# PersiaML/PERSIA

Hardware: AMD Instinct MI355X
Metric: samples/sec (whole node), DLRM-style hybrid training (higher is better)
Workload: dtype bf16; 1 GPU; preset=criteo, model=dlrm 26sparse/13dense dim128, global_batch=8192, rows=100000000, capacity_per_rank=100000000, staleness=8, parallelism=dp1+emb-a2a

## Files before the change

### persia_amd/csrc/dense.hip

```cpp
#include <torch/extension.h>
#include <ATen/hip/HIPContext.h>
#include <hip/hip_runtime.h>
#include <hip/hip_bf16.h>

using bf16 = __hip_bfloat16;
using f32x4 = __attribute__((ext_vector_type(4))) float;
using bf16x8 = __attribute__((ext_vector_type(8))) short;

namespace {

constexpr int BM = 128, BN = 128, BK = 32;
constexpr int PAD = 8;
constexpr int LDK = BK + PAD;

__device__ __forceinline__ float bf2f(short x) {
  union { float f; unsigned u; } v;
  v.u = ((unsigned)(unsigned short)x) << 16;
  return v.f;
}

__device__ __forceinline__ short f2bf(float f) {
  union { float f; unsigned u; } v;
  v.f = f;
  unsigned lsb = (v.u >> 16) & 1;
  v.u += 0x7fff + lsb;
  return (short)(v.u >> 16);
}

template <int ACT, bool STORE_F32, bool TRANS_B, int TBN, int TBK>
__global__ __launch_bounds__(256) void gemm_nt_kernel(
    const bf16* __restrict__ A, const bf16* __restrict__ B,
    const float* __restrict__ bias, void* __restrict__ C, int M, int N,
    int K) {
  constexpr int LK = TBK + PAD;
  __shared__ short lds_a[2][BM * LK];
  __shared__ short lds_b[2][TBN * LK];
  constexpr int WN = TBN / 2;
  constexpr int NFRAG = WN / 16;
  constexpr int PA = BM * TBK / (256 * 8);
  constexpr int PB = TBN * TBK / (256 * 8);
  constexpr int ACPR = TBK / 8;

  const int n_tiles_n = (N + TBN - 1) / TBN;
  const int m0 = (blockIdx.x / n_tiles_n) * BM;
  const int n0 = (blockIdx.x % n_tiles_n) * TBN;

  const int tid = threadIdx.x;
  const int lane = tid % 64;
  const int wave = tid / 64;
  const int wr = wave / 2, wc = wave % 2;
  const int fi = lane & 15;
  const int fk8 = (lane >> 4) * 8;

  f32x4 acc[4][NFRAG] = {};

  auto stage_load = [&](int k0, bf16x8 (&ra)[PA], bf16x8 (&rb)[PB]) {
#pragma unroll
    for (int i = 0; i < PA; ++i) {
      const int p = tid + i * 256;
      const int r = p / ACPR, c8 = (p % ACPR) * 8;
      ra[i] = bf16x8{};
      if (m0 + r < M)
        ra[i] = *(const bf16x8*)(A + (int64_t)(m0 + r) * K + k0 + c8);
    }
#pragma unroll
    for (int i = 0; i < PB; ++i) {
      const int p = tid + i * 256;
      rb[i] = bf16x8{};
      if (!TRANS_B) {
        const int r = p / ACPR, c8 = (p % ACPR) * 8;
        if (n0 + r < N)
          rb[i] = *(const bf16x8*)(B + (int64_t)(n0 + r) * K + k0 + c8);
      } else {
        const int r = p / (TBN / 8), c8 = (p % (TBN / 8)) * 8;
        if (n0 + c8 < N)
          rb[i] = *(const bf16x8*)(B + (int64_t)(k0 + r) * N + n0 + c8);
      }
    }
  };
  auto bswz = [](int n, int k) {
    return n * LK +
           ((((k >> 3) ^ ((n >> 3) & (TBK / 8 - 1))) << 3) | (k & 7));
  };
  auto stage_write = [&](int buf, bf16x8 (&ra)[PA], bf16x8 (&rb)[PB]) {
#pragma unroll
    for (int i = 0; i < PA; ++i) {
      const int p = tid + i * 256;
      const int r = p / ACPR, c8 = (p % ACPR) * 8;
      *(bf16x8*)&lds_a[buf][r * LK + c8] = ra[i];
    }
#pragma unroll
    for (int i = 0; i < PB; ++i) {
      const int p = tid + i * 256;
      if (!TRANS_B) {
        const int r = p / ACPR, c8 = (p % ACPR) * 8;
        *(bf16x8*)&lds_b[buf][bswz(r, c8)] = rb[i];
      } else {
        const int r = p / (TBN / 8), c8 = (p % (TBN / 8)) * 8;
#pragma unroll
        for (int j = 0; j < 8; ++j)
          lds_b[buf][bswz(c8 + j, r)] = rb[i][j];
      }
    }
  };

  int buf = 0;
  {
    bf16x8 ra[PA], rb[PB];
    stage_load(0, ra, rb);
    stage_write(0, ra, rb);
  }
  __syncthreads();

  for (int k0 = 0; k0 < K; k0 += TBK) {
    bf16x8 ra[PA], rb[PB];
    const bool prefetch = k0 + TBK < K;
    if (prefetch) stage_load(k0 + TBK, ra, rb);
#pragma unroll
    for (int kk = 0; kk < TBK; kk += 32) {
#pragma unroll
      for (int am = 0; am < 4; ++am) {
        const bf16x8 a_frag = *(const bf16x8*)
            &lds_a[buf][(wr * 64 + am * 16 + fi) * LK + kk + fk8];
#pragma unroll
        for (int bn = 0; bn < NFRAG; ++bn) {
          const bf16x8 b_frag = *(const bf16x8*)
              &lds_b[buf][bswz(wc * WN + bn * 16 + fi, kk + fk8)];
          acc[am][bn] = __builtin_amdgcn_mfma_f32_16x16x32_bf16(
              a_frag, b_frag, acc[am][bn], 0, 0, 0);
        }
      }
    }
    if (prefetch) stage_write(buf ^ 1, ra, rb);
    buf ^= 1;
    __syncthreads();
  }

#pragma unroll
  for (int am = 0; am < 4; ++am) {
#pragma unroll
    for (int bn = 0; bn < NFRAG; ++bn) {
      const int col = n0 + wc * WN + bn * 16 + fi;
      if (col >= N) continue;
      const float bval = bias ? bias[col] : 0.0f;
#pragma unroll
      for (int r = 0; r < 4; ++r) {
        const int row = m0 + wr * 64 + am * 16 + (lane >> 4) * 4 + r;
        if (row >= M) continue;
        float v = acc[am][bn][r] + bval;
        if (ACT == 1) v = fmaxf(v, 0.0f);
        if (STORE_F32)
          ((float*)C)[(int64_t)row * N + col] = v;
        else
          ((short*)C)[(int64_t)row * N + col] = f2bf(v);
      }
    }
  }
}

using bf16x4t = __attribute__((ext_vector_type(4))) __bf16;

__global__ __launch_bounds__(256) void wgrad_tr_kernel(
    const short* __restrict__ dC, const short* __restrict__ A,
    float* __restrict__ dW, int M, int N, int K, int splitm, int ldw,
    int kmax, int accum) {
  constexpr int MT = 64;
  __shared__ short lds_c[2][8 * MT * 16];
  __shared__ short lds_a[2][8 * MT * 16];
  const int n_tiles_k = K / 128;
  const int tile_id = blockIdx.x / splitm;
  const int m_part = blockIdx.x % splitm;
  const int n0 = (tile_id / n_tiles_k) * 128;
  const int k0 = (tile_id % n_tiles_k) * 128;
  const int tid = threadIdx.x;
  const int wave = tid / 64, lane = tid % 64;
  const int wr = wave / 2, wc = wave % 2;
  const int fi = lane & 15;

  const int m_chunk = ((M + splitm - 1) / splitm + MT - 1) / MT * MT;
  const int m_begin = m_part * m_chunk;
  const int m_end = min(M, m_begin + m_chunk);

  const int s_m = lane >> 1;
  const int s_n8 = (lane & 1) * 8;
  auto stage = [&](int bufi, int m0g) {
#pragma unroll
    for (int c = 0; c < 4; ++c) {
      const int p = wave * 2 + (c >> 1);
      const int mrow = (c & 1) * 32 + s_m;
      const int64_t m_g = (int64_t)(m0g + mrow);
      __builtin_amdgcn_global_load_lds(
          (const uint32_t*)(dC + m_g * N + n0 + p * 16 + s_n8),
          (uint32_t*)&lds_c[bufi][(p * MT + (c & 1) * 32) * 16], 16, 0, 0);
      __builtin_amdgcn_global_load_lds(
          (const uint32_t*)(A + m_g * K + k0 + p * 16 + s_n8),
          (uint32_t*)&lds_a[bufi][(p * MT + (c & 1) * 32) * 16], 16, 0, 0);
    }
  };
  const int t_l4 = (lane & 15) * 4;
  const int t_g8 = (lane >> 4) * 8;
  auto tfrag = [&](const short* img, int p, int ms) {
    const short* b0 = &img[(p * MT + ms + t_g8) * 16 + t_l4];
    bf16x4t lo = __builtin_amdgcn_ds_read_tr16_b64_v4bf16(
        (__attribute__((address_space(3))) bf16x4t*)(void*)const_cast<short*>(b0));
    bf16x4t hi = __builtin_amdgcn_ds_read_tr16_b64_v4bf16(
        (__attribute__((address_space(3))) bf16x4t*)(void*)const_cast<short*>(b0 + 4 * 16));
    bf16x8 r;
#pragma unroll
    for (int j = 0; j < 4; ++j) {
      r[j] = ((const short*)&lo)[j];
      r[4 + j] = ((const short*)&hi)[j];
    }
    return r;
  };

  f32x4 acc[4][4] = {};
  stage(0, m_begin);
  asm volatile("s_waitcnt vmcnt(0)" ::: "memory");
  __builtin_amdgcn_s_barrier();
  int buf = 0;
  for (int m0g = m_begin; m0g < m_end; m0g += MT) {
    if (m0g + MT < m_end) stage(buf ^ 1, m0g + MT);
#pragma unroll
    for (int ms = 0; ms < MT; ms += 32) {
      bf16x8 bfr[4];
#pragma unroll
      for (int bk = 0; bk < 4; ++bk)
        bfr[bk] = tfrag(lds_a[buf], wc * 4 + bk, ms);
#pragma unroll
      for (int an = 0; an < 4; ++an) {
        const bf16x8 afr = tfrag(lds_c[buf], wr * 4 + an, ms);
#pragma unroll
        for (int bk = 0; bk < 4; ++bk)
          acc[an][bk] = __builtin_amdgcn_mfma_f32_16x16x32_bf16(
              afr, bfr[bk], acc[an][bk], 0, 0, 0);
      }
    }
    asm volatile("s_waitcnt vmcnt(0) lgkmcnt(0)" ::: "memory");
    __builtin_amdgcn_s_barrier();
    buf ^= 1;
  }

#pragma unroll
  for (int an = 0; an < 4; ++an) {
#pragma unroll
    for (int bk = 0; bk < 4; ++bk) {
      const int n = n0 + wr * 64 + an * 16 + (lane >> 4) * 4;
      const int k = k0 + wc * 64 + bk * 16 + fi;
      if (k >= kmax) continue;
#pragma unroll
      for (int r = 0; r < 4; ++r) {
        if (accum || splitm > 1)
          atomicAdd(&dW[(int64_t)(n + r) * ldw + k], acc[an][bk][r]);
        else
          dW[(int64_t)(n + r) * ldw + k] = acc[an][bk][r];
      }
    }
  }
}

template <int ACT, bool STORE_F32, int TBN>
__global__ __launch_bounds__(256) void gemm_nt_glds_kernel(
    const bf16* __restrict__ A, const bf16* __restrict__ B,
    const float* __restrict__ bias, void* __restrict__ C, int M, int N,
    int K) {
  constexpr int TBK = 64;
  constexpr int WN = TBN / 2;
  constexpr int NFRAG = WN / 16;
  constexpr int BCH = TBN / 32;
  __shared__ short lds_a[2][128 * TBK];
  __shared__ short lds_b[2][TBN * TBK];
  const int n_tiles_n = N / TBN;
  const int m0 = (blockIdx.x / n_tiles_n) * 128;
  const int n0 = (blockIdx.x % n_tiles_n) * TBN;
  const int tid = threadIdx.x;
  const int lane = tid % 64;
  const int wave = tid / 64;
  const int wr = wave / 2, wc = wave % 2;
  const int fi = lane & 15;
  const int g16 = lane >> 4;

  const int s_rl = lane >> 3;
  const int s_gr = (lane & 7) ^ s_rl;
  auto stage = [&](int bufi, int k0) {
#pragma unroll
    for (int i = 0; i < 4; ++i) {
      const int row = wave * 32 + i * 8 + s_rl;
      const int a_row = min(m0 + row, M - 1);
      __builtin_amdgcn_global_load_lds(
          (const uint32_t*)(A + (int64_t)a_row * K + k0 + s_gr * 8),
          (uint32_t*)&lds_a[bufi][(wave * 32 + i * 8) * TBK], 16, 0, 0);
    }
#pragma unroll
    for (int i = 0; i < BCH; ++i) {
      const int brow = wave * (TBN / 4) + i * 8 + s_rl;
      __builtin_amdgcn_global_load_lds(
          (const uint32_t*)(B + (int64_t)(n0 + brow) * K + k0 + s_gr * 8),
          (uint32_t*)&lds_b[bufi][(wave * (TBN / 4) + i * 8) * TBK], 16, 0, 0);
    }
  };
  auto frag = [&](const short* base, int row, int gr) {
    return *(const bf16x8*)&base[row * TBK + ((gr ^ (row & 7)) << 3)];
  };

  f32x4 acc[4][NFRAG] = {};
  stage(0, 0);
  asm volatile("s_waitcnt vmcnt(0)" ::: "memory");
  __builtin_amdgcn_s_barrier();
  int buf = 0;
  for (int k0 = 0; k0 < K; k0 += TBK) {
    if (k0 + TBK < K) stage(buf ^ 1, k0 + TBK);
#pragma unroll
    for (int kk = 0; kk < 2; ++kk) {
      bf16x8 bfr[NFRAG];
#pragma unroll
      for (int bn = 0; bn < NFRAG; ++bn)
        bfr[bn] = frag(lds_b[buf], wc * WN + bn * 16 + fi, kk * 4 + g16);
#pragma unroll
      for (int am = 0; am < 4; ++am) {
        const bf16x8 afr = frag(lds_a[buf], wr * 64 + am * 16 + fi,
                                kk * 4 + g16);
#pragma unroll
        for (int bn = 0; bn < NFRAG; ++bn)
          acc[am][bn] = __builtin_amdgcn_mfma_f32_16x16x32_bf16(
              afr, bfr[bn], acc[am][bn], 0, 0, 0);
      }
    }
    asm volatile("s_waitcnt vmcnt(0) lgkmcnt(0)" ::: "memory");
    __builtin_amdgcn_s_barrier();
    buf ^= 1;
  }

#pragma unroll
  for (int am = 0; am < 4; ++am) {
#pragma unroll
    for (int bn = 0; bn < NFRAG; ++bn) {
      const int col = n0 + wc * WN + bn * 16 + fi;
      const float bval = bias ? bias[col] : 0.0f;
#pragma unroll
      for (int r = 0; r < 4; ++r) {
        const int row = m0 + wr * 64 + am * 16 + (lane >> 4) * 4 + r;
        if (row >= M) continue;
        float v = acc[am][bn][r] + bval;
        if (ACT == 1) v = fmaxf(v, 0.0f);
        if (STORE_F32)
          ((float*)C)[(int64_t)row * N + col] = v;
        else
          ((short*)C)[(int64_t)row * N + col] = f2bf(v);
      }
    }
  }
}

template <int ACT, bool STORE_F32>
__global__ __launch_bounds__(256) void gemm_nt_glds3_kernel(
    const bf16* __restrict__ A, const bf16* __restrict__ B,
    const float* __restrict__ bias, void* __restrict__ C, int M, int N,
    int K) {
  constexpr int TBK = 64;
  __shared__ short lds_a[3][128 * TBK];
  __shared__ short lds_b[3][128 * TBK];
  const int n_tiles_n = N / 128;
  const int m0 = (blockIdx.x / n_tiles_n) * 128;
  const int n0 = (blockIdx.x % n_tiles_n) * 128;
  const int tid = threadIdx.x;
  const int lane = tid % 64;
  const int wave = tid / 64;
  const int wr = wave / 2, wc = wave % 2;
  const int fi = lane & 15;
  const int g16 = lane >> 4;
  const int s_rl = lane >> 3;
  const int s_gr = (lane & 7) ^ s_rl;
  auto stage = [&](int bufi, int k0) {
#pragma unroll
    for (int i = 0; i < 4; ++i) {
      const int row = wave * 32 + i * 8 + s_rl;
      const int a_row = min(m0 + row, M - 1);
      __builtin_amdgcn_global_load_lds(
          (const uint32_t*)(A + (int64_t)a_row * K + k0 + s_gr * 8),
          (uint32_t*)&lds_a[bufi][(wave * 32 + i * 8) * TBK], 16, 0, 0);
      __builtin_amdgcn_global_load_lds(
          (const uint32_t*)(B + (int64_t)(n0 + row) * K + k0 + s_gr * 8),
          (uint32_t*)&lds_b[bufi][(wave * 32 + i * 8) * TBK], 16, 0, 0);
    }
  };
  auto frag = [&](const short* base, int row, int gr) {
    return *(const bf16x8*)&base[row * TBK + ((gr ^ (row & 7)) << 3)];
  };

  f32x4 acc[4][4] = {};
  const int nt = K / TBK;
  stage(0, 0);
  if (nt > 1) {
    stage(1, TBK);
    asm volatile("s_waitcnt vmcnt(8)" ::: "memory");
  } else {
    asm volatile("s_waitcnt vmcnt(0)" ::: "memory");
  }
  __builtin_amdgcn_s_barrier();
  for (int t = 0; t < nt; ++t) {
    if (t + 2 < nt) stage((t + 2) % 3, (t + 2) * TBK);
    const short* la = lds_a[t % 3];
    const short* lb = lds_b[t % 3];
#pragma unroll
    for (int kk = 0; kk < 2; ++kk) {
      bf16x8 bfr[4];
#pragma unroll
      for (int bn = 0; bn < 4; ++bn)
        bfr[bn] = frag(lb, wc * 64 + bn * 16 + fi, kk * 4 + g16);
#pragma unroll
      for (int am = 0; am < 4; ++am) {
        const bf16x8 afr = frag(la, wr * 64 + am * 16 + fi, kk * 4 + g16);
#pragma unroll
        for (int bn = 0; bn < 4; ++bn)
          acc[am][bn] = __builtin_amdgcn_mfma_f32_16x16x32_bf16(
              afr, bfr[bn], acc[am][bn], 0, 0, 0);
      }
    }
    if (t + 2 < nt)
      asm volatile("s_waitcnt vmcnt(8) lgkmcnt(0)" ::: "memory");
    else
      asm volatile("s_waitcnt vmcnt(0) lgkmcnt(0)" ::: "memory");
    __builtin_amdgcn_s_barrier();
  }

#pragma unroll
  for (int am = 0; am < 4; ++am) {
#pragma unroll
    for (int bn = 0; bn < 4; ++bn) {
      const int col = n0 + wc * 64 + bn * 16 + fi;
      const float bval = bias ? bias[col] : 0.0f;
#pragma unroll
      for (int r = 0; r < 4; ++r) {
        const int row = m0 + wr * 64 + am * 16 + (lane >> 4) * 4 + r;
        if (row >= M) continue;
        float v = acc[am][bn][r] + bval;
        if (ACT == 1) v = fmaxf(v, 0.0f);
        if (STORE_F32)
          ((float*)C)[(int64_t)row * N + col] = v;
        else
          ((short*)C)[(int64_t)row * N + col] = f2bf(v);
      }
    }
  }
}

constexpr int WTM = 64;
constexpr int WLD = WTM + PAD;

__global__ __launch_bounds__(256) void wgrad_kernel(
    const short* __restrict__ dC, const short* __restrict__ A,
    float* __restrict__ dW, int M, int N, int K, int splitm, int ldw,
    int kmax, int accum) {
  __shared__ short lds_dct[2][64 * WLD];
  __shared__ short lds_at[2][64 * WLD];

  const int n_tiles_k = (K + 63) / 64;
  const int tile_id = blockIdx.x / splitm;
  const int m_part = blockIdx.x % splitm;
  const int n0 = (tile_id / n_tiles_k) * 64;
  const int k0 = (tile_id % n_tiles_k) * 64;

  const int tid = threadIdx.x;
  const int wave = tid / 64, lane = tid % 64;
  const int wr = wave / 2, wc = wave % 2;
  const int fi = lane & 15;
  const int fk8 = (lane >> 4) * 8;

  const int m_chunk = ((M + splitm - 1) / splitm + WTM - 1) / WTM * WTM;
  const int m_begin = m_part * m_chunk;
  const int m_end = min(M, m_begin + m_chunk);

  f32x4 acc[2][2] = {};

  const int s_m = tid / 8, s_c8 = (tid % 8) * 8;

  auto wload = [&](int m0, bf16x8 (&v)[2], bf16x8 (&w)[2]) {
#pragma unroll
    for (int h = 0; h < 2; ++h) {
      const int m = m0 + s_m + h * 32;
      v[h] = bf16x8{};
      if (m < M && n0 + s_c8 < N)
        v[h] = *(const bf16x8*)(dC + (int64_t)m * N + n0 + s_c8);
      w[h] = bf16x8{};
      if (m < M && k0 + s_c8 < K)
// ... 41 lines not shown
        }
      }
    }
    if (prefetch) wwrite(buf ^ 1, v, w);
    buf ^= 1;
    __syncthreads();
  }

#pragma unroll
  for (int an = 0; an < 2; ++an) {
#pragma unroll
    for (int bk = 0; bk < 2; ++bk) {
      const int k = k0 + wc * 32 + bk * 16 + fi;
      if (k >= kmax) continue;
#pragma unroll
      for (int r = 0; r < 4; ++r) {
        const int n = n0 + wr * 32 + an * 16 + (lane >> 4) * 4 + r;
        if (n >= N) continue;
        if (accum || splitm > 1)
          atomicAdd(&dW[(int64_t)n * ldw + k], acc[an][bk][r]);
        else
          dW[(int64_t)n * ldw + k] = acc[an][bk][r];
      }
    }
  }
}

__global__ void bce_fwd_kernel(const float* __restrict__ z,
                               const float* __restrict__ y,
                               float* __restrict__ sig,
                               float* __restrict__ loss_sum, int64_t n) {
  const int64_t i = (int64_t)blockIdx.x * blockDim.x + threadIdx.x;
  float l = 0.0f;
  if (i < n) {
    const float zi = z[i], yi = y[i];
    sig[i] = 1.0f / (1.0f + __expf(-zi));
    l = fmaxf(zi, 0.0f) - zi * yi + __logf(1.0f + __expf(-fabsf(zi)));
  }
  __shared__ float part[256];
  part[threadIdx.x] = l;
  __syncthreads();
  for (int s = 128; s > 0; s >>= 1) {
    if (threadIdx.x < s) part[threadIdx.x] += part[threadIdx.x + s];
    __syncthreads();
  }
  if (threadIdx.x == 0) atomicAdd(loss_sum, part[0]);
}

__global__ void bce_bwd_kernel(const float* __restrict__ sig,
                               const float* __restrict__ y,
                               const float* __restrict__ gscale,
                               float* __restrict__ dz, int64_t n) {
  const int64_t i = (int64_t)blockIdx.x * blockDim.x + threadIdx.x;
  if (i >= n) return;
  dz[i] = gscale[0] * (sig[i] - y[i]) / (float)n;
}

__global__ void relu_bwd_kernel(const short* __restrict__ g,
                                const short* __restrict__ out,
                                short* __restrict__ g_eff, int64_t n) {
  const int64_t i = ((int64_t)blockIdx.x * blockDim.x + threadIdx.x) * 8;
  if (i >= n) return;
  bf16x8 gv = *(const bf16x8*)(g + i);
  bf16x8 ov = *(const bf16x8*)(out + i);
  bf16x8 r;
#pragma unroll
  for (int j = 0; j < 8; ++j) r[j] = bf2f(ov[j]) > 0.0f ? gv[j] : (short)0;
  *(bf16x8*)(g_eff + i) = r;
}

__global__ __launch_bounds__(256) void relu_bwd_bias_kernel(
    const short* __restrict__ g, const short* __restrict__ out,
    short* __restrict__ g_eff, float* __restrict__ db, int64_t total8,
    int N) {
  extern __shared__ float lds_col[];
  const int n8 = N / 8;
  for (int i = threadIdx.x; i < N; i += blockDim.x) lds_col[i] = 0.0f;
  __syncthreads();
  const int64_t stride = (int64_t)gridDim.x * blockDim.x;
  int64_t idx = (int64_t)blockIdx.x * blockDim.x + threadIdx.x;
  const int c8 = (int)((idx % n8) * 8);
  float acc[8] = {};
  for (; idx < total8; idx += stride) {
    const bf16x8 gv = *(const bf16x8*)(g + idx * 8);
    const bf16x8 ov = *(const bf16x8*)(out + idx * 8);
    bf16x8 r;
#pragma unroll
    for (int j = 0; j < 8; ++j) {
      r[j] = bf2f(ov[j]) > 0.0f ? gv[j] : (short)0;
      acc[j] += bf2f(r[j]);
    }
    *(bf16x8*)(g_eff + idx * 8) = r;
  }
#pragma unroll
  for (int j = 0; j < 8; ++j) atomicAdd(&lds_col[c8 + j], acc[j]);
  __syncthreads();
  for (int i = threadIdx.x; i < N; i += blockDim.x)
    atomicAdd(&db[i], lds_col[i]);
}

__global__ void bias_grad_kernel(const short* __restrict__ dC,
                                 float* __restrict__ db, int M, int N,
                                 int rows_per_block) {
  const int m_begin = blockIdx.x * rows_per_block;
  const int m_end = min(M, m_begin + rows_per_block);
  for (int col = threadIdx.x; col < N; col += blockDim.x) {
    float acc = 0.0f;
    for (int m = m_begin; m < m_end; ++m) acc += bf2f(dC[(int64_t)m * N + col]);
    atomicAdd(&db[col], acc);
  }
}

__global__ __launch_bounds__(256) void bias_grad_vec_kernel(
    const short* __restrict__ dC, float* __restrict__ db, int64_t total8,
    int N) {
  extern __shared__ float lds_col[];
  const int n8 = N / 8;
  for (int i = threadIdx.x; i < N; i += blockDim.x) lds_col[i] = 0.0f;
  __syncthreads();
  const int64_t stride = (int64_t)gridDim.x * blockDim.x;
  int64_t idx = (int64_t)blockIdx.x * blockDim.x + threadIdx.x;
  const int c8 = (int)((idx % n8) * 8);
  float acc[8] = {};
  constexpr int U = 4;
  for (; idx + 3 * stride < total8; idx += U * stride) {
    bf16x8 v[U];
#pragma unroll
    for (int t = 0; t < U; ++t)
      v[t] = *(const bf16x8*)(dC + (idx + t * stride) * 8);
#pragma unroll
    for (int t = 0; t < U; ++t)
#pragma unroll
      for (int j = 0; j < 8; ++j) acc[j] += bf2f(v[t][j]);
  }
  for (; idx < total8; idx += stride) {
    const bf16x8 v = *(const bf16x8*)(dC + idx * 8);
#pragma unroll
    for (int j = 0; j < 8; ++j) acc[j] += bf2f(v[j]);
  }
#pragma unroll
  for (int j = 0; j < 8; ++j) atomicAdd(&lds_col[c8 + j], acc[j]);
  __syncthreads();
  for (int i = threadIdx.x; i < N; i += blockDim.x)
    atomicAdd(&db[i], lds_col[i]);
}

}


static hipStream_t dcur_stream() {
  return at::hip::getCurrentHIPStream().stream();
}

torch::Tensor gemm_nt_bias_act(torch::Tensor A, torch::Tensor B,
                               torch::Tensor bias, int64_t act,
                               int64_t out_f32, int64_t trans_b) {
  TORCH_CHECK(A.scalar_type() == torch::kBFloat16 &&
              B.scalar_type() == torch::kBFloat16);
  TORCH_CHECK(A.is_contiguous() && B.is_contiguous());
  const int M = (int)A.size(0), K = (int)A.size(1);
  const int N = (int)(trans_b ? B.size(1) : B.size(0));
  TORCH_CHECK((trans_b ? B.size(0) : B.size(1)) == K, "gemm_nt shape mismatch");
  TORCH_CHECK(K % BK == 0, "K must be a multiple of 32 (pad)");
  TORCH_CHECK(N % 8 == 0, "N must be a multiple of 8");
  auto C = torch::empty(
      {M, N},
      torch::TensorOptions()
          .dtype(out_f32 ? torch::kFloat32 : torch::kBFloat16)
          .device(A.device()));
  const int m_tiles = (M + BM - 1) / BM;
  static const bool v2_on = [] {
    const char* e = getenv("PA_GEMM_V2");
    return !e || atoi(e) != 0;
  }();
  const bool v2_shape = v2_on && !trans_b && K % 64 == 0 && M >= 128 &&
                        K >= 256;
  const bool v2_128 = v2_shape && N % 128 == 0 &&
                      (int64_t)m_tiles * (N / 128) >= 400;
  const bool v2_64 = v2_shape && !v2_128 && N % 64 == 0 &&
                     (int64_t)m_tiles * (N / 64) >= 400;
  static const bool v3_on = [] {
    const char* e = getenv("PA_GEMM_V3");
    return e && atoi(e) != 0;
  }();
  if (v3_on && v2_128) {
    const int grid = m_tiles * (N / 128);
    const float* bias_p = bias.numel() ? bias.data_ptr<float>() : nullptr;
#define PA_GEMM3(ACTV, F32V)                                                  \
  hipLaunchKernelGGL((gemm_nt_glds3_kernel<ACTV, F32V>), dim3(grid),          \
                     dim3(256), 0, dcur_stream(),                             \
                     (const bf16*)A.data_ptr(), (const bf16*)B.data_ptr(),    \
                     bias_p, C.data_ptr(), M, N, K)
    if (act == 1) { if (out_f32) PA_GEMM3(1, true); else PA_GEMM3(1, false); }
    else          { if (out_f32) PA_GEMM3(0, true); else PA_GEMM3(0, false); }
#undef PA_GEMM3
    return C;
  }
  if (v2_128 || v2_64) {
    const int tbn = v2_128 ? 128 : 64;
    const int grid = m_tiles * (N / tbn);
    const float* bias_p = bias.numel() ? bias.data_ptr<float>() : nullptr;
#define PA_GEMM2(ACTV, F32V, TBNV)                                            \
  hipLaunchKernelGGL((gemm_nt_glds_kernel<ACTV, F32V, TBNV>), dim3(grid),     \
                     dim3(256), 0, dcur_stream(),                             \
                     (const bf16*)A.data_ptr(), (const bf16*)B.data_ptr(),    \
                     bias_p, C.data_ptr(), M, N, K)
#define PA_GEMM2_T(ACTV, F32V)                                                \
  do {                                                                        \
    if (v2_128) PA_GEMM2(ACTV, F32V, 128);                                    \
    else PA_GEMM2(ACTV, F32V, 64);                                            \
  } while (0)
    if (act == 1) { if (out_f32) PA_GEMM2_T(1, true); else PA_GEMM2_T(1, false); }
    else          { if (out_f32) PA_GEMM2_T(0, true); else PA_GEMM2_T(0, false); }
#undef PA_GEMM2_T
#undef PA_GEMM2
    return C;
  }
  const bool k64 = K % 64 == 0 && N % 64 == 0;
  const bool narrow =
      ((int64_t)m_tiles * ((N + 127) / 128) < 192 && N % 64 == 0) || k64;
  const int tbn = narrow ? 64 : 128;
  const int grid = m_tiles * ((N + tbn - 1) / tbn);
  const float* bias_ptr = bias.numel() ? bias.data_ptr<float>() : nullptr;
  hipStream_t st = dcur_stream();
#define PA_GEMM(ACTV, F32V, TBV, TBNV, TBKV)                                  \
  hipLaunchKernelGGL((gemm_nt_kernel<ACTV, F32V, TBV, TBNV, TBKV>),           \
                     dim3(grid), dim3(256), 0, st, (const bf16*)A.data_ptr(), \
                     (const bf16*)B.data_ptr(), bias_ptr, C.data_ptr(), M, N, \
                     K)
#define PA_GEMM_CFG(ACTV, F32V, TBV)                                          \
  do {                                                                        \
    if (k64) PA_GEMM(ACTV, F32V, TBV, 64, 64);                                \
    else if (narrow) PA_GEMM(ACTV, F32V, TBV, 64, 32);                        \
    else PA_GEMM(ACTV, F32V, TBV, 128, 32);                                   \
  } while (0)
#define PA_GEMM_T(ACTV, F32V)                                                 \
  do {                                                                        \
    if (trans_b) PA_GEMM_CFG(ACTV, F32V, true);                               \
    else PA_GEMM_CFG(ACTV, F32V, false);                                      \
  } while (0)
  if (act == 1) { if (out_f32) PA_GEMM_T(1, true); else PA_GEMM_T(1, false); }
  else          { if (out_f32) PA_GEMM_T(0, true); else PA_GEMM_T(0, false); }
#undef PA_GEMM_T
#undef PA_GEMM_CFG
#undef PA_GEMM
  return C;
}

torch::Tensor relu_bwd_bias(torch::Tensor g, torch::Tensor out,
                            torch::Tensor db) {
  const int64_t M = g.size(0), N = g.size(1);
  TORCH_CHECK(db.scalar_type() == torch::kFloat32 && db.numel() == N);
  const bool pow2 = (N & (N - 1)) == 0 && N >= 8 && N <= 8192;
  TORCH_CHECK(pow2, "relu_bwd_bias: power-of-two N only");
  auto g_eff = torch::empty_like(g);
  const int64_t total8 = M * N / 8;
  const int n8 = (int)(N / 8);
  int blocks = (int)std::min<int64_t>(256, (total8 + 255) / 256);
  if (n8 > 256) blocks = ((blocks + n8 / 256 - 1) / (n8 / 256)) * (n8 / 256);
  hipLaunchKernelGGL(relu_bwd_bias_kernel, dim3(blocks), dim3(256),
                     (int)N * sizeof(float), dcur_stream(),
                     (const short*)g.data_ptr(), (const short*)out.data_ptr(),
                     (short*)g_eff.data_ptr(), db.data_ptr<float>(), total8,
                     (int)N);
  return g_eff;
}

torch::Tensor relu_bwd(torch::Tensor g, torch::Tensor out) {
  auto g_eff = torch::empty_like(g);
  const int64_t n = g.numel();
  TORCH_CHECK(n % 8 == 0);
  const int64_t blocks = (n / 8 + 255) / 256;
  hipLaunchKernelGGL(relu_bwd_kernel,
                     dim3((unsigned)std::min<int64_t>(blocks, 1 << 30)),
                     dim3(256), 0, dcur_stream(), (const short*)g.data_ptr(),
                     (const short*)out.data_ptr(), (short*)g_eff.data_ptr(), n);
  return g_eff;
}

static void bias_grad_launch(torch::Tensor dC, torch::Tensor db) {
  const int M = (int)dC.size(0), N = (int)dC.size(1);
  const bool pow2 = (N & (N - 1)) == 0 && N >= 8 && N <= 8192;
  if (pow2) {
    const int64_t total8 = (int64_t)M * N / 8;
    static const int kBlocks = [] {
      const char* e = getenv("PA_BIAS_BLOCKS");
      return e ? atoi(e) : 96;
    }();
    int blocks = (int)std::min<int64_t>(kBlocks, (total8 + 255) / 256);
    const int n8 = N / 8;
    if (n8 > 256) blocks = ((blocks + n8 / 256 - 1) / (n8 / 256)) * (n8 / 256);
    hipLaunchKernelGGL(bias_grad_vec_kernel, dim3(blocks), dim3(256),
                       N * sizeof(float), dcur_stream(),
                       (const short*)dC.data_ptr(), db.data_ptr<float>(),
                       total8, N);
    return;
  }
  const int rows_per_block = std::max(8, (M + 511) / 512);
  const int blocks = (M + rows_per_block - 1) / rows_per_block;
  hipLaunchKernelGGL(bias_grad_kernel, dim3(blocks), dim3(256), 0,
                     dcur_stream(), (const short*)dC.data_ptr(),
                     db.data_ptr<float>(), M, N, rows_per_block);
}

torch::Tensor bias_grad(torch::Tensor dC) {
  auto db = torch::zeros(
      {dC.size(1)},
      torch::TensorOptions().dtype(torch::kFloat32).device(dC.device()));
  bias_grad_launch(dC, db);
  return db;
}

void bias_grad_into(torch::Tensor dC, torch::Tensor out) {
  TORCH_CHECK(out.scalar_type() == torch::kFloat32 && out.is_contiguous());
  TORCH_CHECK(out.numel() == dC.size(1));
  bias_grad_launch(dC, out);
}

static void wgrad_launch(torch::Tensor dC, torch::Tensor A, torch::Tensor out,
                         int ldw, int kmax, int accum) {
  const int M = (int)dC.size(0), N = (int)dC.size(1), K = (int)A.size(1);
  static const bool tr_on = [] {
    const char* e = getenv("PA_WGRAD_TR");
    return !e || atoi(e) != 0;
  }();
  if (tr_on && M % 64 == 0 && N % 128 == 0 && K % 128 == 0 &&
      (N / 128) * (K / 128) >= 64) {
    const int tiles2 = (N / 128) * (K / 128);
    int splitm = 1;
    while (tiles2 * splitm < 512 && splitm < 64 && (M / (splitm * 2)) >= 64)
      splitm *= 2;
    if (splitm > 1 && !accum) out.zero_();
    hipLaunchKernelGGL(wgrad_tr_kernel, dim3(tiles2 * splitm), dim3(256), 0,
                       dcur_stream(), (const short*)dC.data_ptr(),
                       (const short*)A.data_ptr(), out.data_ptr<float>(), M, N,
                       K, splitm, ldw, kmax, accum);
    return;
  }
  const int tiles = ((N + 63) / 64) * ((K + 63) / 64);
  int splitm = 1;
  while (tiles * splitm < 512 && splitm < 64 && (M / (splitm * 2)) >= 32)
    splitm *= 2;
  if (splitm > 1 && !accum) out.zero_();
  hipLaunchKernelGGL(wgrad_kernel, dim3(tiles * splitm), dim3(256), 0,
                     dcur_stream(), (const short*)dC.data_ptr(),
                     (const short*)A.data_ptr(), out.data_ptr<float>(), M, N,
                     K, splitm, ldw, kmax, accum);
}

torch::Tensor wgrad(torch::Tensor dC, torch::Tensor A) {
  const int N = (int)dC.size(1), K = (int)A.size(1);
  auto dW = torch::empty(
      {N, K}, torch::TensorOptions().dtype(torch::kFloat32).device(A.device()));
  wgrad_launch(dC, A, dW, K, K, 0);
  return dW;
}

void wgrad_into(torch::Tensor dC, torch::Tensor A, torch::Tensor out) {
  TORCH_CHECK(out.scalar_type() == torch::kFloat32 && out.is_contiguous());
  TORCH_CHECK(out.size(0) == dC.size(1) && out.size(1) <= A.size(1));
  wgrad_launch(dC, A, out, (int)out.size(1), (int)out.size(1), 1);
}

std::vector<torch::Tensor> bce_fwd(torch::Tensor z, torch::Tensor y) {
  TORCH_CHECK(z.scalar_type() == torch::kFloat32 && y.scalar_type() == torch::kFloat32);
  const int64_t n = z.numel();
  auto sig = torch::empty_like(z);
  auto loss = torch::zeros({1}, z.options());
  hipLaunchKernelGGL(bce_fwd_kernel, dim3((unsigned)((n + 255) / 256)),
                     dim3(256), 0, dcur_stream(), z.data_ptr<float>(),
                     y.data_ptr<float>(), sig.data_ptr<float>(),
                     loss.data_ptr<float>(), n);
  loss.div_((double)n);
  return {loss.squeeze(0), sig};
}

torch::Tensor bce_bwd(torch::Tensor sig, torch::Tensor y, torch::Tensor g) {
  const int64_t n = sig.numel();
  auto dz = torch::empty_like(sig);
  hipLaunchKernelGGL(bce_bwd_kernel, dim3((unsigned)((n + 255) / 256)),
                     dim3(256), 0, dcur_stream(), sig.data_ptr<float>(),
                     y.data_ptr<float>(), g.data_ptr<float>(),
                     dz.data_ptr<float>(), n);
  return dz;
}

void init_dense(pybind11::module_& m) {
  m.def("gemm_nt_bias_act", &gemm_nt_bias_act,
        "bf16 MFMA GEMM (A @ B^T) with fused bias+activation");
  m.def("relu_bwd", &relu_bwd, "g * (out > 0)");
  m.def("relu_bwd_bias", &relu_bwd_bias,
        "relu backward fused with the bias column-sum accumulation");
  m.def("bce_fwd", &bce_fwd, "fused BCE-with-logits forward (loss + sigmoid cache)");
  m.def("bce_bwd", &bce_bwd, "fused BCE-with-logits backward");
  m.def("bias_grad", &bias_grad, "column-sum bias gradient");
  m.def("wgrad", &wgrad, "dW = dC^T @ A (f32 out)");
  m.def("wgrad_into", &wgrad_into,
        "dW accumulated straight into a flat f32 grad slot");
  m.def("bias_grad_into", &bias_grad_into,
        "bias grad accumulated straight into a flat f32 grad slot");
}
```

### persia_amd/ops/dense.py

```python
from typing import List, Optional

import torch
import torch.nn as nn
import torch.nn.functional as F


def _wgrad_via_blas() -> bool:
    import os

    return os.environ.get("PA_FUSED_WGRAD", "own") == "blas"


def _pad32(x: torch.Tensor, dim: int, mult: int = 128) -> torch.Tensor:
    k = x.shape[dim]
    pad = (-k) % mult
    if pad == 0:
        return x
    padding = [0, 0] * (x.dim() - 1 - dim) + [0, pad]
    return F.pad(x, padding)


class FusedLinearFn(torch.autograd.Function):
    @staticmethod
    def forward(ctx, x, weight, bias, act: int):
        from persia_amd.ops import native

        C = native()
        x_bf = _pad32(x.to(torch.bfloat16), 1).contiguous()
        w_bf = _pad32(weight.to(torch.bfloat16), 1).contiguous()
        out = C.gemm_nt_bias_act(x_bf, w_bf, bias.float(), act, 0, 0)
        ctx.save_for_backward(x_bf, w_bf, out)
        ctx.act = act
        ctx.k = x.shape[1]
        ctx.kw = weight.shape[1]
        ctx.w_dtype = weight.dtype
        ctx.b_dtype = bias.dtype
        ctx.w_side = getattr(weight, "_sideband_grad", None)
        ctx.b_side = getattr(bias, "_sideband_grad", None)
        return out

    @staticmethod
    def backward(ctx, g):
        from persia_amd.ops import native

        C = native()
        x_bf, w_bf, out = ctx.saved_tensors
        g = g.to(torch.bfloat16).contiguous()
        N = g.shape[1]
        pow2 = N >= 8 and (N & (N - 1)) == 0
        if ctx.act == 1 and pow2 and ctx.b_side is not None:
            g = C.relu_bwd_bias(g, out, ctx.b_side)
            db = None
        else:
            if ctx.act == 1:
                g = C.relu_bwd(g, out)
            if ctx.b_side is not None:
                C.bias_grad_into(g, ctx.b_side)
                db = None
            else:
                db = C.bias_grad(g)
                if db.dtype != ctx.b_dtype:
                    db = db.to(ctx.b_dtype)
        if w_bf.shape[0] >= 1024 and w_bf.shape[1] >= 1024:
            dx = C.gemm_nt_bias_act(
                g, w_bf.t().contiguous(), torch.empty(0, device=g.device),
                0, 0, 0,
            )
        else:
            dx = C.gemm_nt_bias_act(
                g, w_bf, torch.empty(0, device=g.device), 0, 0, 1
            )
        if dx.shape[1] != ctx.k:
            dx = dx[:, : ctx.k]
        if ctx.w_side is not None:
            C.wgrad_into(g, x_bf, ctx.w_side)
            dw = None
        elif _wgrad_via_blas():
            dw = torch.matmul(g.t(), x_bf).to(ctx.w_dtype)
        else:
            dw = C.wgrad(g, x_bf)
            if dw.dtype != ctx.w_dtype:
                dw = dw.to(ctx.w_dtype)
        if dw is not None and dw.shape[1] != ctx.kw:
            dw = dw[:, : ctx.kw].contiguous()
        return dx, dw, db, None


class FusedLinear(nn.Module):
    def __init__(self, in_features: int, out_features: int, relu: bool = True,
                 bias: bool = True):
        super().__init__()
        assert out_features % 32 == 0, "FusedLinear needs out_features % 32 == 0"
        self.in_features = in_features
        self.out_features = out_features
        self.relu = relu
        self.weight = nn.Parameter(torch.empty(out_features, in_features))
        if bias:
            self.bias = nn.Parameter(torch.zeros(out_features))
        else:
            self.register_buffer("bias", torch.zeros(out_features))
        nn.init.kaiming_uniform_(self.weight, a=5 ** 0.5)

    def _apply(self, fn, recurse=True):
        r = super()._apply(fn, recurse)
        if self.bias.dtype != torch.float32:
            if isinstance(self.bias, nn.Parameter):
                self.bias.data = self.bias.data.float()
                if self.bias.grad is not None:
                    self.bias.grad = self.bias.grad.float()
            else:
                self.bias = self.bias.float()
        return r

    def forward(self, x):
        return FusedLinearFn.apply(x, self.weight, self.bias, 1 if self.relu else 0)


class FusedMLP(nn.Module):

    def __init__(self, sizes: List[int], last_relu: bool = False):
        super().__init__()
        layers: List[nn.Module] = []
        for i in range(len(sizes) - 1):
            is_last = i == len(sizes) - 2
            relu = (not is_last) or last_relu
            if sizes[i + 1] % 32 == 0:
                layers.append(FusedLinear(sizes[i], sizes[i + 1], relu=relu))
            else:
                lin = nn.Linear(sizes[i], sizes[i + 1])
                layers.append(lin if not relu else nn.Sequential(lin, nn.ReLU()))
        self.layers = nn.ModuleList(layers)

    def forward(self, x):
        for l in self.layers:
            if not isinstance(l, FusedLinear):
                w = next(l.parameters(), None)
                if w is not None and x.dtype != w.dtype:
                    x = x.to(w.dtype)
            x = l(x)
        return x


class FusedBCEFn(torch.autograd.Function):

    @staticmethod
    def forward(ctx, logits, label):
        from persia_amd.ops import native

        C = native()
        loss, sig = C.bce_fwd(logits.float().contiguous(),
                              label.float().contiguous())
        ctx.save_for_backward(sig, label)
        ctx.in_dtype = logits.dtype
        return loss

    @staticmethod
    def backward(ctx, g):
        from persia_amd.ops import native

        C = native()
        sig, label = ctx.saved_tensors
        dz = C.bce_bwd(sig, label.float(), g.reshape(1).float().contiguous())
        if dz.dtype != ctx.in_dtype:
            dz = dz.to(ctx.in_dtype)
        return dz, None


def fused_bce_with_logits(logits: torch.Tensor, label: torch.Tensor) -> torch.Tensor:
    return FusedBCEFn.apply(logits, label)
```

Measured before the change: 6.927 million samples/s.

## Fuse ReLU-backward mask and bias-grad reduction into dgrad GEMM epilogue across MLP chains

Adds a DRELU epilogue to the GEMM kernels that applies the previous layer's ReLU mask (taken from the saved bf16 input activation) and accumulates bias-gradient column sums through LDS and atomics. This lets a single kernel produce the masked dx for the next layer down. A new FusedChainFn autograd function runs consecutive FusedLinear layers as one chain, so the separate relu_bwd/bias_grad passes over the gradient are no longer needed. The intent is to cut extra memory passes and kernel launches in the MLP backward. The costs are a heavier epilogue with extra mask loads and atomics, a bias gradient summed from bf16-rounded values, and new dispatch plumbing.

Measured after the change: 7.734 million samples/s, median of 6. +11.7%, better.

```diff
diff --git a/persia_amd/csrc/dense.hip b/persia_amd/csrc/dense.hip
--- a/persia_amd/csrc/dense.hip
+++ b/persia_amd/csrc/dense.hip
@@ -27,11 +27,75 @@
   return (short)(v.u >> 16);
 }
 
-template <int ACT, bool STORE_F32, bool TRANS_B, int TBN, int TBK>
+template <int TBN, int NFRAG, int FG>
+__device__ __forceinline__ void drelu_bias_epilogue(
+    const f32x4 (&acc)[4][NFRAG], short* __restrict__ C,
+    const short* __restrict__ mask, float* __restrict__ db, float* part,
+    int M, int N, int n_bias, int m0, int n0, int wr, int wc, int lane,
+    int tid) {
+  constexpr int WN = TBN / 2;
+  const int fi = lane & 15;
+  const int rl0 = wr * 64 + (lane >> 4) * 4;
+  const int cl0 = wc * WN + fi;
+  const int rl_max = M - 1 - m0, cl_max = N - 1 - n0;
+  const int64_t origin = ((int64_t)m0 * N + n0) * 2;
+  const char* mtile = (const char*)mask + origin;
+  char* ctile = (char*)C + origin;
+  float csum[NFRAG] = {};
+#pragma unroll
+  for (int f0 = 0; f0 < 4 * NFRAG; f0 += FG) {
+    short mk[FG][4];
+#pragma unroll
+    for (int f = 0; f < FG; ++f)
+#pragma unroll
+      for (int r = 0; r < 4; ++r) {
+        const int am = (f0 + f) / NFRAG, bn = (f0 + f) % NFRAG;
+        const int rl = min(rl0 + am * 16 + r, rl_max);
+        const int cl = min(cl0 + bn * 16, cl_max);
+        mk[f][r] = *(const short*)(mtile + (unsigned)(rl * N + cl) * 2u);
+      }
+    short sv[FG][4];
+#pragma unroll
+    for (int f = 0; f < FG; ++f)
+#pragma unroll
+      for (int r = 0; r < 4; ++r) {
+        const int am = (f0 + f) / NFRAG, bn = (f0 + f) % NFRAG;
+        const bool ok = rl0 + am * 16 + r <= rl_max && cl0 + bn * 16 <= cl_max;
+        float v = acc[am][bn][r] + 0.0f;
+        v = bf2f(mk[f][r]) > 0.0f ? v : 0.0f;
+        sv[f][r] = f2bf(v);
+        csum[bn] += ok ? bf2f(sv[f][r]) : 0.0f;
+      }
+#pragma unroll
+    for (int f = 0; f < FG; ++f)
+#pragma unroll
+      for (int r = 0; r < 4; ++r) {
+        const int am = (f0 + f) / NFRAG, bn = (f0 + f) % NFRAG;
+        const int rl = rl0 + am * 16 + r;
+        const int cl = cl0 + bn * 16;
+        if (rl <= rl_max && cl <= cl_max)
+          *(short*)(ctile + (unsigned)(rl * N + cl) * 2u) = sv[f][r];
+      }
+  }
+#pragma unroll
+  for (int bn = 0; bn < NFRAG; ++bn) {
+    float s = csum[bn];
+    s += __shfl_xor(s, 16);
+    s += __shfl_xor(s, 32);
+    if (lane < 16) part[wr * TBN + wc * WN + bn * 16 + fi] = s;
+  }
+  __syncthreads();
+  if (tid < TBN && n0 + tid < n_bias)
+    atomicAdd(&db[n0 + tid], part[tid] + part[TBN + tid]);
+}
+
+template <int ACT, bool STORE_F32, bool TRANS_B, int TBN, int TBK,
+          bool DRELU = false>
 __global__ __launch_bounds__(256) void gemm_nt_kernel(
     const bf16* __restrict__ A, const bf16* __restrict__ B,
     const float* __restrict__ bias, void* __restrict__ C, int M, int N,
-    int K) {
+    int K, const short* __restrict__ mask, float* __restrict__ db,
+    int n_bias) {
   constexpr int LK = TBK + PAD;
   __shared__ short lds_a[2][BM * LK];
   __shared__ short lds_b[2][TBN * LK];
@@ -136,6 +200,12 @@
     __syncthreads();
   }
 
+  if constexpr (DRELU) {
+    drelu_bias_epilogue<TBN, NFRAG, (TBK == 64 ? 4 * NFRAG : 1)>(
+        acc, (short*)C, mask, db, (float*)&lds_a[0][0], M, N, n_bias, m0, n0,
+        wr, wc, lane, tid);
+    return;
+  }
 #pragma unroll
   for (int am = 0; am < 4; ++am) {
 #pragma unroll
@@ -259,11 +329,12 @@
   }
 }
 
-template <int ACT, bool STORE_F32, int TBN>
+template <int ACT, bool STORE_F32, int TBN, bool DRELU = false>
 __global__ __launch_bounds__(256) void gemm_nt_glds_kernel(
     const bf16* __restrict__ A, const bf16* __restrict__ B,
     const float* __restrict__ bias, void* __restrict__ C, int M, int N,
-    int K) {
+    int K, const short* __restrict__ mask, float* __restrict__ db,
+    int n_bias) {
   constexpr int TBK = 64;
   constexpr int WN = TBN / 2;
   constexpr int NFRAG = WN / 16;
@@ -331,6 +402,12 @@
     buf ^= 1;
   }
 
+  if constexpr (DRELU) {
+    drelu_bias_epilogue<TBN, NFRAG, 4 * NFRAG>(acc, (short*)C, mask, db,
+                                       (float*)&lds_a[0][0], M, N, n_bias,
+                                       m0, n0, wr, wc, lane, tid);
+    return;
+  }
 #pragma unroll
   for (int am = 0; am < 4; ++am) {
 #pragma unroll
@@ -678,22 +755,12 @@
   return at::hip::getCurrentHIPStream().stream();
 }
 
-torch::Tensor gemm_nt_bias_act(torch::Tensor A, torch::Tensor B,
-                               torch::Tensor bias, int64_t act,
-                               int64_t out_f32, int64_t trans_b) {
-  TORCH_CHECK(A.scalar_type() == torch::kBFloat16 &&
-              B.scalar_type() == torch::kBFloat16);
-  TORCH_CHECK(A.is_contiguous() && B.is_contiguous());
-  const int M = (int)A.size(0), K = (int)A.size(1);
-  const int N = (int)(trans_b ? B.size(1) : B.size(0));
-  TORCH_CHECK((trans_b ? B.size(0) : B.size(1)) == K, "gemm_nt shape mismatch");
-  TORCH_CHECK(K % BK == 0, "K must be a multiple of 32 (pad)");
-  TORCH_CHECK(N % 8 == 0, "N must be a multiple of 8");
-  auto C = torch::empty(
-      {M, N},
-      torch::TensorOptions()
-          .dtype(out_f32 ? torch::kFloat32 : torch::kBFloat16)
-          .device(A.device()));
+enum GemmFamily { kGemmV1 = 0, kGemmGlds = 1, kGemmGlds3 = 2 };
+struct GemmPlan {
+  int family, tbn, tbk, grid;
+};
+
+static GemmPlan gemm_plan(int M, int N, int K, bool trans_b) {
   const int m_tiles = (M + BM - 1) / BM;
   static const bool v2_on = [] {
     const char* e = getenv("PA_GEMM_V2");
@@ -709,68 +776,126 @@
     const char* e = getenv("PA_GEMM_V3");
     return e && atoi(e) != 0;
   }();
-  if (v3_on && v2_128) {
-    const int grid = m_tiles * (N / 128);
-    const float* bias_p = bias.numel() ? bias.data_ptr<float>() : nullptr;
-#define PA_GEMM3(ACTV, F32V)                                                  \
-  hipLaunchKernelGGL((gemm_nt_glds3_kernel<ACTV, F32V>), dim3(grid),          \
-                     dim3(256), 0, dcur_stream(),                             \
-                     (const bf16*)A.data_ptr(), (const bf16*)B.data_ptr(),    \
-                     bias_p, C.data_ptr(), M, N, K)
-    if (act == 1) { if (out_f32) PA_GEMM3(1, true); else PA_GEMM3(1, false); }
-    else          { if (out_f32) PA_GEMM3(0, true); else PA_GEMM3(0, false); }
-#undef PA_GEMM3
-    return C;
-  }
+  if (v3_on && v2_128) return {kGemmGlds3, 128, 64, m_tiles * (N / 128)};
   if (v2_128 || v2_64) {
     const int tbn = v2_128 ? 128 : 64;
-    const int grid = m_tiles * (N / tbn);
-    const float* bias_p = bias.numel() ? bias.data_ptr<float>() : nullptr;
-#define PA_GEMM2(ACTV, F32V, TBNV)                                            \
-  hipLaunchKernelGGL((gemm_nt_glds_kernel<ACTV, F32V, TBNV>), dim3(grid),     \
-                     dim3(256), 0, dcur_stream(),                             \
-                     (const bf16*)A.data_ptr(), (const bf16*)B.data_ptr(),    \
-                     bias_p, C.data_ptr(), M, N, K)
-#define PA_GEMM2_T(ACTV, F32V)                                                \
-  do {                                                                        \
-    if (v2_128) PA_GEMM2(ACTV, F32V, 128);                                    \
-    else PA_GEMM2(ACTV, F32V, 64);                                            \
-  } while (0)
-    if (act == 1) { if (out_f32) PA_GEMM2_T(1, true); else PA_GEMM2_T(1, false); }
-    else          { if (out_f32) PA_GEMM2_T(0, true); else PA_GEMM2_T(0, false); }
-#undef PA_GEMM2_T
-#undef PA_GEMM2
-    return C;
+    return {kGemmGlds, tbn, 64, m_tiles * (N / tbn)};
   }
   const bool k64 = K % 64 == 0 && N % 64 == 0;
   const bool narrow =
       ((int64_t)m_tiles * ((N + 127) / 128) < 192 && N % 64 == 0) || k64;
   const int tbn = narrow ? 64 : 128;
-  const int grid = m_tiles * ((N + tbn - 1) / tbn);
-  const float* bias_ptr = bias.numel() ? bias.data_ptr<float>() : nullptr;
+  return {kGemmV1, tbn, k64 ? 64 : 32, m_tiles * ((N + tbn - 1) / tbn)};
+}
+
+template <int ACT, bool F32, bool DRELU>
+static void gemm_launch(const GemmPlan& p, bool trans_b, const void* A,
+                        const void* B, const float* bias, void* C, int M,
+                        int N, int K, const short* mask, float* db,
+                        int n_bias) {
   hipStream_t st = dcur_stream();
-#define PA_GEMM(ACTV, F32V, TBV, TBNV, TBKV)                                  \
-  hipLaunchKernelGGL((gemm_nt_kernel<ACTV, F32V, TBV, TBNV, TBKV>),           \
-                     dim3(grid), dim3(256), 0, st, (const bf16*)A.data_ptr(), \
-                     (const bf16*)B.data_ptr(), bias_ptr, C.data_ptr(), M, N, \
-                     K)
-#define PA_GEMM_CFG(ACTV, F32V, TBV)                                          \
+#define PA_GEMM_ARGS                                                          \
+  dim3(p.grid), dim3(256), 0, st, (const bf16*)A, (const bf16*)B, bias, C, M, \
+      N, K, mask, db, n_bias
+  if constexpr (!DRELU) {
+    if (p.family == kGemmGlds3) {
+      hipLaunchKernelGGL((gemm_nt_glds3_kernel<ACT, F32>), dim3(p.grid),
+                         dim3(256), 0, st, (const bf16*)A, (const bf16*)B,
+                         bias, C, M, N, K);
+      return;
+    }
+  }
+  if (p.family != kGemmV1) {
+    if (p.tbn == 128)
+      hipLaunchKernelGGL((gemm_nt_glds_kernel<ACT, F32, 128, DRELU>),
+                         PA_GEMM_ARGS);
+    else
+      hipLaunchKernelGGL((gemm_nt_glds_kernel<ACT, F32, 64, DRELU>),
+                         PA_GEMM_ARGS);
+    return;
+  }
+#define PA_GEMM_CFG(TBV)                                                      \
   do {                                                                        \
-    if (k64) PA_GEMM(ACTV, F32V, TBV, 64, 64);                                \
-    else if (narrow) PA_GEMM(ACTV, F32V, TBV, 64, 32);                        \
-    else PA_GEMM(ACTV, F32V, TBV, 128, 32);                                   \
+    if (p.tbk == 64)                                                          \
+      hipLaunchKernelGGL((gemm_nt_kernel<ACT, F32, TBV, 64, 64, DRELU>),      \
+                         PA_GEMM_ARGS);                                       \
+    else if (p.tbn == 64)                                                     \
+      hipLaunchKernelGGL((gemm_nt_kernel<ACT, F32, TBV, 64, 32, DRELU>),      \
+                         PA_GEMM_ARGS);                                       \
+    else                                                                      \
+      hipLaunchKernelGGL((gemm_nt_kernel<ACT, F32, TBV, 128, 32, DRELU>),     \
+                         PA_GEMM_ARGS);                                       \
   } while (0)
-#define PA_GEMM_T(ACTV, F32V)                                                 \
-  do {                                                                        \
-    if (trans_b) PA_GEMM_CFG(ACTV, F32V, true);                               \
-    else PA_GEMM_CFG(ACTV, F32V, false);                                      \
-  } while (0)
-  if (act == 1) { if (out_f32) PA_GEMM_T(1, true); else PA_GEMM_T(1, false); }
-  else          { if (out_f32) PA_GEMM_T(0, true); else PA_GEMM_T(0, false); }
-#undef PA_GEMM_T
+  if (trans_b) PA_GEMM_CFG(true);
+  else PA_GEMM_CFG(false);
 #undef PA_GEMM_CFG
-#undef PA_GEMM
+#undef PA_GEMM_ARGS
+}
+
+static void gemm_check_operands(const torch::Tensor& A, const torch::Tensor& B,
+                                int64_t trans_b, int& M, int& N, int& K) {
+  TORCH_CHECK(A.scalar_type() == torch::kBFloat16 &&
+              B.scalar_type() == torch::kBFloat16);
+  TORCH_CHECK(A.is_contiguous() && B.is_contiguous());
+  M = (int)A.size(0);
+  K = (int)A.size(1);
+  N = (int)(trans_b ? B.size(1) : B.size(0));
+  TORCH_CHECK((trans_b ? B.size(0) : B.size(1)) == K, "gemm_nt shape mismatch");
+  TORCH_CHECK(K % BK == 0, "K must be a multiple of 32 (pad)");
+  TORCH_CHECK(N % 8 == 0, "N must be a multiple of 8");
+}
+
+torch::Tensor gemm_nt_bias_act(torch::Tensor A, torch::Tensor B,
+                               torch::Tensor bias, int64_t act,
+                               int64_t out_f32, int64_t trans_b) {
+  int M, N, K;
+  gemm_check_operands(A, B, trans_b, M, N, K);
+  auto C = torch::empty(
+      {M, N},
+      torch::TensorOptions()
+          .dtype(out_f32 ? torch::kFloat32 : torch::kBFloat16)
+          .device(A.device()));
+  const GemmPlan p = gemm_plan(M, N, K, trans_b != 0);
+  const float* bias_p = bias.numel() ? bias.data_ptr<float>() : nullptr;
+#define PA_GEMM_GO(ACTV, F32V)                                                \
+  gemm_launch<ACTV, F32V, false>(p, trans_b != 0, A.data_ptr(), B.data_ptr(), \
+                                 bias_p, C.data_ptr(), M, N, K, nullptr,      \
+                                 nullptr, 0)
+  if (act == 1) { if (out_f32) PA_GEMM_GO(1, true); else PA_GEMM_GO(1, false); }
+  else          { if (out_f32) PA_GEMM_GO(0, true); else PA_GEMM_GO(0, false); }
+#undef PA_GEMM_GO
   return C;
+}
+
+torch::Tensor dgrad_drelu_bias(torch::Tensor g, torch::Tensor W,
+                               int64_t trans_b, torch::Tensor mask,
+                               torch::Tensor db, int64_t n_bias) {
+  int M, N, K;
+  gemm_check_operands(g, W, trans_b, M, N, K);
+  TORCH_CHECK(mask.scalar_type() == torch::kBFloat16 && mask.is_contiguous() &&
+                  mask.dim() == 2 && mask.size(0) == M && mask.size(1) == N,
+              "dgrad_drelu_bias: mask must be contiguous bf16 [M, N]");
+  TORCH_CHECK(db.scalar_type() == torch::kFloat32 && db.is_contiguous());
+  TORCH_CHECK(n_bias >= 0 && n_bias <= N && db.numel() >= n_bias,
+              "dgrad_drelu_bias: n_bias out of range");
+  TORCH_CHECK(N <= (1 << 23), "dgrad_drelu_bias: N too large");
+  TORCH_CHECK(mask.device() == g.device() && db.device() == g.device());
+  auto dx = torch::empty(
+      {M, N}, torch::TensorOptions().dtype(torch::kBFloat16).device(g.device()));
+  const GemmPlan p = gemm_plan(M, N, K, trans_b != 0);
+  gemm_launch<0, false, true>(p, trans_b != 0, g.data_ptr(), W.data_ptr(),
+                              nullptr, dx.data_ptr(), M, N, K,
+                              (const short*)mask.data_ptr(),
+                              db.data_ptr<float>(), (int)n_bias);
+  return dx;
+}
+
+std::string gemm_nt_config(int64_t M, int64_t N, int64_t K, int64_t trans_b) {
+  const GemmPlan p = gemm_plan((int)M, (int)N, (int)K, trans_b != 0);
+  if (p.family == kGemmV1)
+    return "v1:" + std::to_string(p.tbn) + "x" + std::to_string(p.tbk);
+  return std::string(p.family == kGemmGlds3 ? "glds3:" : "glds:") +
+         std::to_string(p.tbn);
 }
 
 torch::Tensor relu_bwd_bias(torch::Tensor g, torch::Tensor out,
@@ -914,6 +1039,10 @@
 void init_dense(pybind11::module_& m) {
   m.def("gemm_nt_bias_act", &gemm_nt_bias_act,
         "bf16 MFMA GEMM (A @ B^T) with fused bias+activation");
+  m.def("dgrad_drelu_bias", &dgrad_drelu_bias,
+        "dgrad GEMM with fused ReLU-backward mask + bias-grad column sums");
+  m.def("gemm_nt_config", &gemm_nt_config,
+        "kernel family / tile config the GEMM dispatch picks for a shape");
   m.def("relu_bwd", &relu_bwd, "g * (out > 0)");
   m.def("relu_bwd_bias", &relu_bwd_bias,
         "relu backward fused with the bias column-sum accumulation");
diff --git a/persia_amd/ops/dense.py b/persia_amd/ops/dense.py
--- a/persia_amd/ops/dense.py
+++ b/persia_amd/ops/dense.py
@@ -18,6 +18,55 @@
         return x
     padding = [0, 0] * (x.dim() - 1 - dim) + [0, pad]
     return F.pad(x, padding)
+
+
+def _fused_drelu() -> bool:
+    import os
+
+    return os.environ.get("PA_FUSED_DRELU", "1") != "0"
+
+
+def _own_bias_grad(C, g, out, act, b_side, b_dtype):
+    N = g.shape[1]
+    pow2 = N >= 8 and (N & (N - 1)) == 0
+    if act == 1 and pow2 and b_side is not None:
+        return C.relu_bwd_bias(g, out, b_side), None
+    if act == 1:
+        g = C.relu_bwd(g, out)
+    if b_side is not None:
+        C.bias_grad_into(g, b_side)
+        return g, None
+    db = C.bias_grad(g)
+    if db.dtype != b_dtype:
+        db = db.to(b_dtype)
+    return g, db
+
+
+def _dgrad(C, g, w_bf, mask=None, db=None, n_bias=0):
+    if w_bf.shape[0] >= 1024 and w_bf.shape[1] >= 1024:
+        w_op, trans_b = w_bf.t().contiguous(), 0
+    else:
+        w_op, trans_b = w_bf, 1
+    if mask is None:
+        return C.gemm_nt_bias_act(
+            g, w_op, torch.empty(0, device=g.device), 0, 0, trans_b
+        )
+    return C.dgrad_drelu_bias(g, w_op, trans_b, mask, db, n_bias)
+
+
+def _wgrad(C, g, x_bf, w_side, w_dtype, kw):
+    if w_side is not None:
+        C.wgrad_into(g, x_bf, w_side)
+        return None
+    if _wgrad_via_blas():
+        dw = torch.matmul(g.t(), x_bf).to(w_dtype)
+    else:
+        dw = C.wgrad(g, x_bf)
+        if dw.dtype != w_dtype:
+            dw = dw.to(w_dtype)
+    if dw.shape[1] != kw:
+        dw = dw[:, :kw].contiguous()
+    return dw
 
 
 class FusedLinearFn(torch.autograd.Function):
@@ -46,44 +95,83 @@
         C = native()
         x_bf, w_bf, out = ctx.saved_tensors
         g = g.to(torch.bfloat16).contiguous()
-        N = g.shape[1]
-        pow2 = N >= 8 and (N & (N - 1)) == 0
-        if ctx.act == 1 and pow2 and ctx.b_side is not None:
-            g = C.relu_bwd_bias(g, out, ctx.b_side)
-            db = None
-        else:
-            if ctx.act == 1:
-                g = C.relu_bwd(g, out)
-            if ctx.b_side is not None:
-                C.bias_grad_into(g, ctx.b_side)
-                db = None
-            else:
-                db = C.bias_grad(g)
-                if db.dtype != ctx.b_dtype:
-                    db = db.to(ctx.b_dtype)
-        if w_bf.shape[0] >= 1024 and w_bf.shape[1] >= 1024:
-            dx = C.gemm_nt_bias_act(
-                g, w_bf.t().contiguous(), torch.empty(0, device=g.device),
-                0, 0, 0,
-            )
-        else:
-            dx = C.gemm_nt_bias_act(
-                g, w_bf, torch.empty(0, device=g.device), 0, 0, 1
-            )
-        if dx.shape[1] != ctx.k:
-            dx = dx[:, : ctx.k]
-        if ctx.w_side is not None:
-            C.wgrad_into(g, x_bf, ctx.w_side)
-            dw = None
-        elif _wgrad_via_blas():
-            dw = torch.matmul(g.t(), x_bf).to(ctx.w_dtype)
-        else:
-            dw = C.wgrad(g, x_bf)
-            if dw.dtype != ctx.w_dtype:
-                dw = dw.to(ctx.w_dtype)
-        if dw is not None and dw.shape[1] != ctx.kw:
-            dw = dw[:, : ctx.kw].contiguous()
+        g, db = _own_bias_grad(C, g, out, ctx.act, ctx.b_side, ctx.b_dtype)
+        dx = None
+        if ctx.needs_input_grad[0]:
+            dx = _dgrad(C, g, w_bf)
+            if dx.shape[1] != ctx.k:
+                dx = dx[:, : ctx.k]
+        dw = _wgrad(C, g, x_bf, ctx.w_side, ctx.w_dtype, ctx.kw)
         return dx, dw, db, None
+
+
+class FusedChainFn(torch.autograd.Function):
+
+    @staticmethod
+    def forward(ctx, x, acts, *params):
+        from persia_amd.ops import native
+
+        C = native()
+        weights, biases = params[0::2], params[1::2]
+        saved, widths = [], []
+        h = x
+        for w, b, act in zip(weights, biases, acts):
+            x_bf = _pad32(h.to(torch.bfloat16), 1).contiguous()
+            w_bf = _pad32(w.to(torch.bfloat16), 1).contiguous()
+            widths.append(h.shape[1])
+            h = C.gemm_nt_bias_act(x_bf, w_bf, b.float(), act, 0, 0)
+            saved += [x_bf, w_bf]
+        ctx.save_for_backward(*saved, h)
+        ctx.acts = tuple(acts)
+        ctx.widths = widths
+        ctx.kws = [w.shape[1] for w in weights]
+        ctx.w_dtypes = [w.dtype for w in weights]
+        ctx.b_dtypes = [b.dtype for b in biases]
+        ctx.w_sides = [getattr(w, "_sideband_grad", None) for w in weights]
+        ctx.b_sides = [getattr(b, "_sideband_grad", None) for b in biases]
+        return h
+
+    @staticmethod
+    def backward(ctx, g):
+        from persia_amd.ops import native
+
+        C = native()
+        *saved, out = ctx.saved_tensors
+        L = len(ctx.acts)
+        g = g.to(torch.bfloat16).contiguous()
+        grads = [None] * (2 * L)
+        dx = None
+        g, grads[2 * L - 1] = _own_bias_grad(
+            C, g, out, ctx.acts[-1], ctx.b_sides[-1], ctx.b_dtypes[-1]
+        )
+        for i in range(L - 1, -1, -1):
+            x_bf, w_bf = saved[2 * i], saved[2 * i + 1]
+            dx = None
+            if i > 0 and ctx.acts[i - 1] == 1:
+                n_prev = ctx.widths[i]
+                db = ctx.b_sides[i - 1]
+                fresh = db is None
+                if fresh:
+                    db = torch.zeros(n_prev, dtype=torch.float32,
+                                     device=g.device)
+                dx = _dgrad(C, g, w_bf, mask=x_bf, db=db, n_bias=n_prev)
+                if fresh:
+                    if db.dtype != ctx.b_dtypes[i - 1]:
+                        db = db.to(ctx.b_dtypes[i - 1])
+                    grads[2 * i - 1] = db
+            elif i > 0 or ctx.needs_input_grad[0]:
+                dx = _dgrad(C, g, w_bf)
+            grads[2 * i] = _wgrad(C, g, x_bf, ctx.w_sides[i], ctx.w_dtypes[i],
+                                  ctx.kws[i])
+            if dx is not None and dx.shape[1] != ctx.widths[i]:
+                dx = dx[:, : ctx.widths[i]]
+            if i > 0:
+                g = dx.contiguous()
+                if ctx.acts[i - 1] != 1:
+                    g, grads[2 * i - 1] = _own_bias_grad(
+                        C, g, x_bf, 0, ctx.b_sides[i - 1], ctx.b_dtypes[i - 1]
+                    )
+        return (dx, None, *grads)
 
 
 class FusedLinear(nn.Module):
@@ -132,12 +220,29 @@
         self.layers = nn.ModuleList(layers)
 
     def forward(self, x):
-        for l in self.layers:
-            if not isinstance(l, FusedLinear):
-                w = next(l.parameters(), None)
-                if w is not None and x.dtype != w.dtype:
-                    x = x.to(w.dtype)
+        layers = list(self.layers)
+        fuse = _fused_drelu()
+        i = 0
+        while i < len(layers):
+            l = layers[i]
+            if isinstance(l, FusedLinear):
+                j = i + 1
+                while fuse and j < len(layers) and isinstance(layers[j], FusedLinear):
+                    j += 1
+                if j - i > 1:
+                    run = layers[i:j]
+                    params = [p for m in run for p in (m.weight, m.bias)]
+                    acts = tuple(1 if m.relu else 0 for m in run)
+                    x = FusedChainFn.apply(x, acts, *params)
+                else:
+                    x = l(x)
+                i = j
+                continue
+            w = next(l.parameters(), None)
+            if w is not None and x.dtype != w.dtype:
+                x = x.to(w.dtype)
             x = l(x)
+            i += 1
         return x
 
 
```
